# Kamino666/S2VT-video-caption

Hardware: AMD Instinct MI355X
Metric: training frames/sec (whole node) (higher is better)
Workload: dtype f32; 1 GPU; BASELINE configs[1]: S2VT train step, B=64 per GPU x 1 GPU, 80x4096 feats, hidden=embed=1000, vocab=12000, fp32, Adam; global_batch=64, frames=80, parallelism=dp1

## Files before the change

### s2vt-video-caption_amd/csrc/api_train.hip

```cpp
#include "api_internal.h"

namespace s2vt {

struct TrainWS : TrainBufs {
    float* colsum_c;
    float* ce_alpha;
    unsigned int *psync_a, *psync_b;
    unsigned short *xw1, *xw2, *xh1, *xh2;
    int64_t xkp;
    bool xfwd;
    unsigned short *xwt1, *xwt2;
    float *xpart1, *xpart2;
    int xnslots; int64_t xpslot, xhp;
    size_t bytes;
};

static TrainWS carve_train(const s2vt_dims& d, void* base) {
    const size_t B = d.B, L = d.L, H = d.H, E = d.E, V = d.V, T = 2 * L - 1;
    Carver c{reinterpret_cast<char*>(base), 0, 0};
    TrainWS w;
    w.bsum1 = c.take<float>(4 * H);
    w.bsum2 = c.take<float>(4 * H);
    w.x1 = c.take<float>(L * B * H);
    w.s1 = c.take<float>(T * B * 4 * H);
    w.h1 = c.take<float>(T * B * H);
    w.c1 = c.take<float>(T * B * H);
    w.s2 = c.take<float>(T * B * 4 * H);
    w.h2 = c.take<float>(T * B * H);
    w.c2 = c.take<float>(T * B * H);
    w.tok = c.take<int32_t>((L - 1) * B);
    w.embws = c.take<int>(embedding_grad_ws_ints((int64_t)(L - 1) * B, (int)d.V));
    w.err = c.take<int>(4);
    w.psync_a = c.take<unsigned int>(lstm_persist_sync_bytes() / sizeof(unsigned int));
    w.psync_b = c.take<unsigned int>(lstm_persist_sync_bytes() / sizeof(unsigned int));
    w.xkp = (H <= 1024) ? (int64_t)((H + 63) / 64 * 64) : 0;
    w.xfwd = w.xkp > 0 && gemm_mode() == 3 && B % 64 == 0 && pipe_block() > 0 && persist_x3_fwd_on();
    w.xw1 = c.take<unsigned short>(w.xfwd ? 3 * 4 * H * w.xkp : 0);
    w.xw2 = c.take<unsigned short>(w.xfwd ? 3 * 4 * H * w.xkp : 0);
    w.xh1 = c.take<unsigned short>(w.xfwd ? 3 * T * B * w.xkp : 0);
    w.xh2 = c.take<unsigned short>(w.xfwd ? 3 * T * B * w.xkp : 0);
    {
        const bool can = w.xkp > 0 && B % 32 == 0 && pipe_block() > 0 && option(O_PERSIST_X3_BWD) != 0 && persist_on() &&
                         (option(O_PERSIST_X3_BWD) == 1 || B * cdiv((int)H, 16) / 32 * 2 <= 256);
        const size_t maxblk = (size_t)pipe_block() < T ? (size_t)pipe_block() : T;
        w.xnslots = can ? (int)maxblk + 1 : 0;
        w.xhp = (int64_t)((H + 15) / 16 * 16);
        w.xpslot = can ? (int64_t)lstm_seq_bwd_x3_part_slot_floats((int)B, (int)H) : 0;
        w.xwt1 = c.take<unsigned short>(can ? 3 * (size_t)w.xkp * 4 * w.xhp : 0);
        w.xwt2 = c.take<unsigned short>(can ? 3 * (size_t)w.xkp * 4 * w.xhp : 0);
        w.xpart1 = c.take<float>((size_t)w.xnslots * w.xpslot);
        w.xpart2 = c.take<float>((size_t)w.xnslots * w.xpslot);
    }
    w.wt1 = c.take<float>(H * 4 * H);
    w.wt2 = c.take<float>(H * 4 * H);
    w.dh1 = c.take<float>(T * B * H);
    w.dh2dec = c.take<float>((L - 1) * B * H);
    w.dx1 = c.take<float>(L * B * H);
    w.de = c.take<float>((L - 1) * B * E);
    w.dc1 = c.take<float>(B * H);
    w.dc2 = c.take<float>(B * H);
    w.ce_alpha = c.take<float>(64);
    size_t cs = 2 * colsum_partial_floats((int64_t)T * B, (int)(4 * H));
    size_t cs2 = colsum_partial_floats((int64_t)(L - 1) * B, (int)V);
    size_t cs3 = colsum_partial_floats((int64_t)L * B, (int)H);
    const size_t csm = cs > cs2 ? (cs > cs3 ? cs : cs3) : (cs2 > cs3 ? cs2 : cs3);
    w.colsum_a = c.take<float>(csm);
    w.colsum_b = c.take<float>(csm);
    w.colsum_c = c.take<float>(csm);
    w.gws_floats = gemm_ws_floats(d);
    w.gws_a = c.take<float>(w.gws_floats);
    w.gws_b = c.take<float>(w.gws_floats);
    w.bytes = align_up(c.off, 256);
    return w;
}

static hipEvent_t g_grad_ev[2] = {nullptr, nullptr};
static bool g_grad_ev_set[2] = {false, false};
static int g_bwd_persist_launches = 0, g_bwd_group0_after = 0;
void backward_order_reset() { g_bwd_persist_launches = g_bwd_group0_after = 0; }
int grads_ready(int group, hipStream_t s) {
    if (group == 0) {
        g_bwd_group0_after = g_bwd_persist_launches;
        cu_reserve_window(true);
    }
    if (!g_grad_ev[group]) S2VT_HIP(hipEventCreateWithFlags(&g_grad_ev[group], hipEventDisableTiming));
    if (!graph_capturing()) S2VT_HIP(hipEventRecord(g_grad_ev[group], s));
    g_grad_ev_set[group] = true;
    return 0;
}

struct PlaneWS {
    PB feats, wf, x1, wih1, h1, we, wv, emb, h2r, wo, whh1, whh2;
    PB dlog, woT, wvT, weT, wih1T, dg2, dg1, whh1T, whh2T;
    PB h2decB;
    size_t bytes;
};

static PlaneWS carve_planes(const s2vt_dims& d, int planes, void* base) {
    const size_t B = d.B, L = d.L, F = d.F, H = d.H, E = d.E, V = d.V, T = 2 * L - 1, R = (L - 1) * B;
    Carver c{reinterpret_cast<char*>(base), 0, 0};
    auto mk = [&](size_t rows, size_t k) { return take_planes(c, rows, k, planes); };
    PlaneWS w;
    w.feats = mk(B * L, F);   w.wf = mk(H, F);       w.x1 = mk(L * B, H);    w.wih1 = mk(4 * H, H);
    w.h1 = mk(T * B, H);      w.we = mk(4 * H, E);   w.wv = mk(4 * H, H);    w.emb = mk(R, E);
    w.h2r = mk(T * B, H);     w.wo = mk(V, H);
    if (planes == 1) {
        w.whh1 = mk(4 * H, H); w.whh2 = mk(4 * H, H); w.whh1T = mk(H, 4 * H); w.whh2T = mk(H, 4 * H);
    }
    w.dlog = mk(R, V);        w.woT = mk(H, V);
    w.wvT = mk(H, 4 * H);     w.weT = mk(E, 4 * H);  w.wih1T = mk(H, 4 * H);
    w.dg2 = mk(T * B, 4 * H); w.dg1 = mk(T * B, 4 * H);
    w.h2decB = mk(R, H);
    w.bytes = align_up(c.off, 256);
    return w;
}

struct FwdRecord { s2vt_dims d; int gemm_mode, planes, persist, blk; bool dlog_ready; };
static RecordTable<FwdRecord> g_fwd_records;
static void record_forward(const void* ws, const s2vt_dims& d, bool planes) {
    g_fwd_records.put(ws, FwdRecord{d, gemm_mode(), planes ? train_planes() : 0, persist_bits(), pipe_block(), false});
}
static int check_forward_record(const void* ws, const s2vt_dims& d, bool planes, bool* dlog_ready = nullptr) {
    FwdRecord r;
    S2VT_REQUIRE(g_fwd_records.take(ws, &r), "s2vt_train_backward: no s2vt_train_forward has run on this workspace");
    if (dlog_ready) *dlog_ready = r.dlog_ready;
    S2VT_REQUIRE(memcmp(&r.d, &d, sizeof(d)) == 0, "s2vt_train_backward: dims differ from the forward that filled this workspace");
    S2VT_REQUIRE(r.gemm_mode == gemm_mode() && r.planes == (planes ? train_planes() : 0) && r.persist == persist_bits() && r.blk == pipe_block(),
                 "s2vt_train_backward: the forward ran with gemm mode %d / recurrence options %d / pipeline block %d, now %d / %d / %d: the "
                 "workspace layout differs (do not change gemm_mode / persist / persist_x3_fwd / persist_x3_bwd / pipe_block "
                 "between a forward and its backward)", r.gemm_mode, r.persist, r.blk, gemm_mode(), persist_bits(), pipe_block());
    return 0;
}

static void key_options(std::vector<uint64_t>& key) {
    for (int i = 0; i < O_COUNT; ++i) key.push_back((uint64_t)(uint32_t)option(i));
    key.push_back((uint64_t)(uint32_t)cu_plan_cap_current());
    key.push_back((uint64_t)g_lane_delay_lanes);
    key.push_back((uint64_t)g_lane_delay_us);
}

struct BpttDone {
    int bias_chunk = 64;
    int hh1_t0 = 0;
    long word_grads_ev = -1;
    long demb_ev = -1;
};

struct TrainDriver : Lanes {
    const s2vt_params* p; const s2vt_grads* g; const TrainWS& w; const PlaneWS& q;
    const float* out_mask; float* logits;
    const int B, L, F, H, E, V, T, R, blk;
    const int64_t BH, B4H;
    const bool bf;
    const bool emit;
    std::vector<int> bd;
    TrainDriver(const s2vt_dims* d, const s2vt_params* p_, const s2vt_grads* g_, const TrainWS& w_, const PlaneWS& q_,
                const float* out_mask_, float* logits_)
        : p(p_), g(g_), w(w_), q(q_), out_mask(out_mask_), logits(logits_), B(d->B), L(d->L), F(d->F), H(d->H), E(d->E), V(d->V),
          T(2 * d->L - 1), R((d->L - 1) * d->B), blk(pipe_block()), BH((int64_t)d->B * d->H), B4H(4 * (int64_t)d->B * d->H),
          bf(q_.h1.planes == 1), emit(d->H % 8 == 0) {}
    int open_lanes(hipStream_t caller) { return open(caller, w.gws_a, w.gws_b, w.gws_floats, w.colsum_a, w.colsum_b); }
    void set_bounds(bool persistent) { bd = pipe_bounds(T, L, persistent ? balanced_block(L, blk) : blk); }

    int zero_k16(const PB& img, size_t first, size_t elems) {
        S2VT_HIP(hipMemset2DAsync(img.p + first, (size_t)64 * img.ld * 2, 0, elems * 2, (size_t)(T * B / 64), st));
        return 0;
    }
    int vid_half_gemm(const Lane& ln, int t0, int t1) {
        const bool cap = t0 >= L;
        return pgemm(ln, (t1 - t0) * B, 4 * H, H, q.h1, t0 * B, 0, q.wv, 0, 0, w.s2 + t0 * B4H, 4 * H, ID, cap ? nullptr : w.bsum2, cap);
    }
    int logits_gemm(const Lane& ln, int first_step) {
        const PB* a = &q.h2r;
        int a0 = L * B, rc;
        if (out_mask) {
            if ((rc = mul_vectors(ln.s, w.h2 + (int64_t)L * B * H, out_mask, w.dh2dec, (int64_t)R * H))) return rc;
            a = &q.h2decB; a0 = 0;
            if ((rc = psplit(ln, *a, a0, w.dh2dec, H, ID, R, H))) return rc;
        }
        return pgemm(ln, R - first_step * B, V, H, *a, a0 + first_step * B, 0, q.wo, 0, 0, logits + (int64_t)first_step * V, V, perm(B, L - 1),
                     p->out_b, false);
    }
    int fwd_x3_persistent(int f_cus, int tenths, int gxe_c);
    int fwd_bf16_persistent();
    int fwd_two_lanes();

    int split_dg_block(const Lane& ln, int layer, int t0, int t1, bool want_planes) {
        const PB& dg = layer == 2 ? q.dg2 : q.dg1;
        const float* in = (layer == 2 ? w.s2 : w.s1) + t0 * B4H;
        float* colpart = (layer == 2 ? w.colsum_a : w.colsum_b) + (int64_t)(t0 * B / 64) * 4 * H;
        return want_planes ? pdual(ln, in, 4 * H, ID, (t1 - t0) * B, 4 * H, &dg, t0 * B, nullptr, t0 * B, colpart)
                           : pcolpart(ln, dg.planes, in, 4 * H, ID, (t1 - t0) * B, 4 * H, colpart);
    }
    int dh1_gemm(const Lane& ln, int t0, int t1) {
        return pgemm(ln, (t1 - t0) * B, H, 4 * H, q.dg2, t0 * B, 0, q.wvT, 0, 0, w.dh1 + t0 * BH, H, ID, nullptr, false);
    }
    int word_weight_grads(const Lane& ln) {
        int rc;
        if ((rc = pgemm_tt(ln, 4 * H, H, (T - 1) * B, q.dg2, B, q.h2r, 0, g->word_w_hh, H, ID, nullptr, false))) return rc;
        if ((rc = pgemm_tt(ln, 4 * H, H, T * B, q.dg2, 0, q.h1, 0, g->word_w_ih + E, E + H, ID, nullptr, false))) return rc;
        return pgemm_tt(ln, 4 * H, E, R, q.dg2, L * B, q.emb, 0, g->word_w_ih, E + H, ID, nullptr, false);
    }
    int demb_gemm(const Lane& ln) { return pgemm(ln, R, E, 4 * H, q.dg2, L * B, 0, q.weT, 0, 0, w.de, E, ID, nullptr, false); }
    SeqBwdX3Args bwd_x3_args(int layer, int t0, int t1) {
        const bool word = layer == 2;
        SeqBwdX3Args a = word ? persist_bwd_x3_args(T, t0, t1, B, H, w.xkp, w.xhp, w.xwt2, w.dh2dec, L, w.c2, w.s2, w.dc2, w.xpart2, w.xpslot,
                                                    w.xnslots, w.psync_a, w.err + 1)
                              : persist_bwd_x3_args(T, t0, t1, B, H, w.xkp, w.xhp, w.xwt1, w.dh1, 0, w.c1, w.s1, w.dc1, w.xpart1, w.xpslot,
                                                    w.xnslots, w.psync_b, w.err + 1);
        if (emit) {
            a.dgp = word ? q.dg2.p : q.dg1.p; a.lddgp = word ? q.dg2.ld : q.dg1.ld;
            a.colpart = word ? w.colsum_a : w.colsum_b; a.skip_dg = 1;
        }
        return a;
    }
    int x3_bptt_begin();
    int bptt_x3_one_layer(int corun_cus, int corun_k, BpttDone* done);
    int bptt_x3_two_layer(int corun_cus, int corun_k, BpttDone* done);
    int bptt_bf16_persistent();
    int bptt_two_lanes();
};

int TrainDriver::fwd_x3_persistent(int f_cus, int tenths, int gxe_c) {
    int rc;
    if ((rc = hand(sx, st))) return rc;
    const int nb = (int)bd.size() - 1;
    for (const PB* img : {&q.h1, &q.h2r})
        if ((rc = zero_k16_tail(st, *img, H, (size_t)T * B))) return rc;
    int lg_c = (nb >= 2 && !out_mask) ? (L - 1) * ((2 * tenths + 1) / 3) / 10 : 0;
    if (lg_c > bd[nb - 1] - L) lg_c = bd[nb - 1] - L > 0 ? bd[nb - 1] - L : 0;
    for (int k = 0; k <= nb; ++k) {
        const bool hv = k < nb, hw = k >= 1;
        const bool co_first = k == 0 && nb >= 2 && gxe_c > 0, co_last = k == nb && lg_c > 0;
        if ((co_first || co_last) && (rc = hand(st, sx))) return rc;
        {
        ProfScope ps(st, K_STEP_FWD, (hv ? bd[k + 1] - bd[k] : 0) + (hw ? bd[k] - bd[k - 1] : 0));
        SeqFwdX3Args av, aw;
        if (hv) av = persist_fwd_x3_args(bd[k], bd[k + 1], B, H, T, w.xkp, w.s1, L, w.bsum1, w.xw1, w.xh1, w.h1, w.c1, w.psync_a, w.err + 1);
        if (hw) aw = persist_fwd_x3_args(bd[k - 1], bd[k], B, H, T, w.xkp, w.s2, T, w.bsum2, w.xw2, w.xh2, w.h2, w.c2, w.psync_b, w.err + 1);
        av.hblk = q.h1.p; av.ldhblk = q.h1.ld;
        aw.hblk = q.h2r.p; aw.ldhblk = q.h2r.ld;
        if (hv && hw) rc = lstm_seq_fwd_x3_persist2(st, av, &aw);
        else rc = lstm_seq_fwd_x3_persist2(st, hv ? av : aw, nullptr);
        }
        if (rc) return rc;
        if (co_first || co_last) {
            {
                CuPlanCap cap(f_cus);
                if (co_first)
                    rc = pgemm(lb, gxe_c, 4 * H, E, q.emb, R - gxe_c, 0, q.we, 0, 0, w.s2 + (int64_t)L * B4H + (int64_t)(R - gxe_c) * 4 * H, 4 * H,
                               ID, w.bsum2, false);
                else
                    rc = pgemm(lb, lg_c * B, V, H, q.h2r, L * B, 0, q.wo, 0, 0, logits, V, perm(B, L - 1), p->out_b, false);
            }
            if (rc || (rc = hand(sx, st))) return rc;
        }
        if (hv && (rc = vid_half_gemm(la, bd[k], bd[k + 1]))) return rc;
    }
    return logits_gemm(la, lg_c);
}

int TrainDriver::fwd_bf16_persistent() {
    int rc;
    if ((rc = hand(sx, st))) return rc;
    const int nb = (int)bd.size() - 1;
    for (int k = 0; k <= nb; ++k) {
        const bool hv = k < nb, hw = k >= 1;
        SeqFwdBf16Args av, aw;
        if (hv) av = persist_fwd_args(bd[k], bd[k + 1], B, H, w.s1, L, w.bsum1, q.whh1, q.h1, w.h1, w.c1, w.psync_a, w.err + 1);
        if (hw) aw = persist_fwd_args(bd[k - 1], bd[k], B, H, w.s2, T, w.bsum2, q.whh2, q.h2r, w.h2, w.c2, w.psync_b, w.err + 1);
        {
            ProfScope ps(st, K_STEP_FWD, (hv ? bd[k + 1] - bd[k] : 0) + (hw ? bd[k] - bd[k - 1] : 0));
            if (hv && hw) rc = lstm_seq_fwd_bf16_persist2(st, av, &aw);
            else rc = lstm_seq_fwd_bf16_persist2(st, hv ? av : aw, nullptr);
            if (rc) return rc;
        }
        if (hv && (rc = vid_half_gemm(la, bd[k], bd[k + 1]))) return rc;
    }
    return logits_gemm(la, 0);
}

int TrainDriver::fwd_two_lanes() {
    int rc;
    for (size_t k = 0; k + 1 < bd.size(); ++k) {
        const int t0 = bd[k], t1 = bd[k + 1];
        rc = bf ? seq_fwd_bf16(st, t0, t1, B, H, w.s1, L, w.bsum1, q.whh1, q.h1, w.h1, w.c1)
                : seq_fwd(st, t0, t1, B, H, w.s1, L, w.bsum1, p->vid_w_hh, w.h1, w.c1, true);
        if (rc) return rc;
        if ((rc = hand(st, sx))) return rc;
        if ((rc = pdual(lb, w.h1 + t0 * BH, H, ID, (t1 - t0) * B, H, bf ? nullptr : &q.h1, t0 * B, nullptr, t0 * B, nullptr))) return rc;
        if ((rc = vid_half_gemm(lb, t0, t1))) return rc;
        rc = bf ? seq_fwd_bf16(sx, t0, t1, B, H, w.s2, T, w.bsum2, q.whh2, q.h2r, w.h2, w.c2)
// ... 8 lines not shown
static int train_forward_x3(const s2vt_dims* d, const s2vt_params* p, const float* feats, const int64_t* targets,
                            int64_t targets_ld, float* logits, const TrainWS& w, const PlaneWS& q, hipStream_t st,
                            const float* out_mask) {
    TrainDriver x(d, p, nullptr, w, q, out_mask, logits);
    const int B = x.B, L = x.L, F = x.F, H = x.H, E = x.E, V = x.V, T = x.T, R = x.R;
    const int64_t B4H = x.B4H;
    int rc;
    if ((rc = x.open_lanes(st))) return rc;
    const hipStream_t sx = x.sx;
    const Lane &la = x.la, &lb = x.lb;
    const bool bf = x.bf;
    if ((rc = bias_sums(st, p, H, w.bsum1, w.bsum2))) return rc;
    if ((rc = fill_zero(st, w.err, 4 * sizeof(int)))) return rc;
    if ((rc = targets_to_time_major(st, targets, B, L - 1, targets_ld, V, w.tok, w.err))) return rc;
    if (bf) {
        if ((rc = zero_pad_cols_u16(st, q.h1.p, (int64_t)T * B, q.h1.ld, H, q.h1.kpad))) return rc;
        if ((rc = zero_pad_cols_u16(st, q.h2r.p, (int64_t)T * B, q.h2r.ld, H, q.h2r.kpad))) return rc;
        if ((rc = pdual(la, p->vid_w_hh, H, ID, 4 * H, H, &q.whh1, 0, &q.whh1T, 0, nullptr))) return rc;
    }
    if ((rc = x.hand(st, sx))) return rc;
    if (bf && (rc = pdual(lb, p->word_w_hh, H, ID, 4 * H, H, &q.whh2, 0, &q.whh2T, 0, nullptr))) return rc;
    RecKind kind = train_recurrence_plan(B, H).fwd;
    if (kind == REC_X3_PERSIST && !w.xfwd) kind = REC_PER_STEP;
    if (kind == REC_BF16_PERSIST && !persist_fwd_ok(B, H, q.whh1, q.h1)) kind = REC_PER_STEP;
    const bool px3_fwd = kind == REC_X3_PERSIST;
    if (px3_fwd) {
        if ((rc = split3_rows(sx, p->vid_w_hh, H, 4 * H, H, (int)w.xkp, w.xw1, 4 * (int64_t)H * w.xkp))) return rc;
        if ((rc = split3_rows(sx, p->word_w_hh, H, 4 * H, H, (int)w.xkp, w.xw2, 4 * (int64_t)H * w.xkp))) return rc;
    }
    if ((rc = pdual(lb, p->word_w_ih, E + H, ID, 4 * H, E, &q.we, 0, &q.weT, 0, nullptr))) return rc;
    if ((rc = pdual(lb, p->word_w_ih + E, E + H, ID, 4 * H, H, &q.wv, 0, &q.wvT, 0, nullptr))) return rc;
    if ((rc = pdual(lb, p->out_w, H, ID, V, H, &q.wo, 0, &q.woT, 0, nullptr))) return rc;
    if ((rc = pdual(lb, p->emb_w, E, gather(w.tok), R, E, &q.emb, 0, nullptr, 0, nullptr))) return rc;
    const int f_wgs = px3_fwd ? lstm_seq_fwd_x3_persist_single_workgroups(B, H) : 0;
    const int f_cus = f_wgs > 0 ? (planned_compute_units() - f_wgs - 2) / 8 * 8 : 0;
    const bool stages3 = px3_fwd && pipe_bounds(T, L, balanced_block(L, x.blk)).size() >= 3;
    const int tenths = (stages3 && sx != st && f_cus >= 64 && R >= 2560 && B % 64 == 0) ? option(O_CORUN) : 0;
    const int gxe_c = (R / 64 * (2 * tenths < 8 ? 2 * tenths : 8) / 10) * 64;
    if ((rc = pgemm(lb, R - gxe_c, 4 * H, E, q.emb, 0, 0, q.we, 0, 0, w.s2 + (int64_t)L * B4H, 4 * H, ID, w.bsum2, false))) return rc;
    if ((rc = psplit(la, q.feats, 0, feats, F, ID, B * L, F))) return rc;
    if ((rc = psplit(la, q.wf, 0, p->feat_w, F, ID, H, F))) return rc;
    if ((rc = pdual(la, p->vid_w_ih, H, ID, 4 * H, H, &q.wih1, 0, &q.wih1T, 0, nullptr))) return rc;
    if ((rc = pgemm(la, B * L, H, F, q.feats, 0, 0, q.wf, 0, 0, w.x1, H, perm(L, B), p->feat_b, false))) return rc;
    if ((rc = pdual(la, w.x1, H, ID, L * B, H, &q.x1, 0, nullptr, 0, nullptr))) return rc;
    if ((rc = pgemm(la, L * B, 4 * H, H, q.x1, 0, 0, q.wih1, 0, 0, w.s1, 4 * H, ID, w.bsum1, false))) return rc;
    x.set_bounds(kind != REC_PER_STEP);
    switch (kind) {
    case REC_X3_PERSIST: return x.fwd_x3_persistent(f_cus, tenths, gxe_c);
    case REC_BF16_PERSIST: return x.fwd_bf16_persistent();
    default: return x.fwd_two_lanes();
    }
}

int TrainDriver::x3_bptt_begin() {
    int rc;
    if ((rc = split3_wt(st, w.wt2, H, (int)w.xkp, (int)w.xhp, w.xwt2, w.xkp * 4 * w.xhp))) return rc;
    if ((rc = split3_wt(sx, w.wt1, H, (int)w.xkp, (int)w.xhp, w.xwt1, w.xkp * 4 * w.xhp))) return rc;
    if ((rc = hand(sx, st))) return rc;
    if (emit && q.dg2.kpad > 4 * H) {
        const size_t kc0 = (size_t)(4 * H / 16);
        for (const PB* img : {&q.dg2, &q.dg1}) {
            if ((rc = zero_k16_tail(st, *img, 4 * H, (size_t)T * B))) return rc;
            if (4 * H % 16)
                for (int pl = 0; pl < 3; ++pl)
                    if ((rc = zero_k16(*img, kc0 * K16_REC_ELEMS + (pl * 2 + 1) * K16_HALF_ELEMS, K16_HALF_ELEMS))) return rc;
        }
    }
    return 0;
}

int TrainDriver::bptt_x3_one_layer(int corun_cus, int corun_k, BpttDone* done) {
    int rc;
    const int nb = (int)bd.size() - 1;
    if ((rc = hand(st, sx))) return rc;
    int wo_r = 0;
    auto wo_part = [&]() -> int {
        if (wo_r >= R) return 0;
        int kk = corun_k < R - wo_r ? corun_k : R - wo_r;
        if (R - wo_r - kk < 512) kk = R - wo_r;
        const int r = pgemm_tt(lb, V, H, kk, q.dlog, wo_r, q.h2decB, wo_r, g->out_w, H, ID, nullptr, wo_r > 0);
        wo_r += kk;
        return r;
    };
    std::vector<long> dh1_done((size_t)nb);
    long wo_done = 0;
    {
        CuPlanCap cap(corun_cus);
        for (int k = nb - 1; k >= 0; --k) {
            const int t0 = bd[k], t1 = bd[k + 1];
            {
                ProfScope ps(st, K_STEP_BWD, t1 - t0);
                if ((rc = lstm_seq_bwd_x3_persist2(st, bwd_x3_args(2, t0, t1), nullptr))) return rc;
                ++g_bwd_persist_launches;
            }
            if ((rc = wo_part())) return rc;
            if ((rc = hand(st, sx))) return rc;
            if (!emit && (rc = split_dg_block(lb, 2, t0, t1, true))) return rc;
            if ((rc = dh1_gemm(lb, t0, t1))) return rc;
            if ((rc = record(sx, &dh1_done[(size_t)k]))) return rc;
        }
        while (wo_r < R)
            if ((rc = wo_part())) return rc;
        if ((rc = record(sx, &wo_done))) return rc;
        if ((rc = word_weight_grads(lb))) return rc;
        if ((rc = record(sx, &done->word_grads_ev))) return rc;
        if ((rc = demb_gemm(lb))) return rc;
        if ((rc = record(sx, &done->demb_ev))) return rc;
    }
    const int kc = nb / 2;
    const int hh1_t0 = nb >= 4 ? bd[kc] : 0;
    for (int k = nb - 1; k >= 0; --k) {
        const int t0 = bd[k], t1 = bd[k + 1];
        if ((rc = wait(st, dh1_done[(size_t)k]))) return rc;
        ProfScope ps(st, K_STEP_BWD, t1 - t0);
        if ((rc = lstm_seq_bwd_x3_persist2(st, bwd_x3_args(1, t0, t1), nullptr))) return rc;
        ++g_bwd_persist_launches;
        if (!emit && (rc = split_dg_block(la, 1, t0, t1, true))) return rc;
        if (hh1_t0 > 0 && k == kc) {
            if ((rc = hand(st, sx))) return rc;
            CuPlanCap cap(corun_cus);
            if ((rc = pgemm_tt(lb, 4 * H, H, (T - hh1_t0) * B, q.dg1, hh1_t0 * B, q.h1, (hh1_t0 - 1) * B, g->vid_w_hh, H, ID, nullptr, false))) return rc;
        }
    }
    done->bias_chunk = emit ? 32 : 64;
    done->hh1_t0 = hh1_t0;
    if ((rc = wait(st, wo_done))) return rc;
    if ((rc = grads_ready(0, st))) return rc;
    return hand(st, sx);
}

int TrainDriver::bptt_x3_two_layer(int corun_cus, int corun_k, BpttDone* done) {
    int rc;
    const int nb = (int)bd.size() - 1;
    for (int k = nb - 1; k >= -1; --k) {
        const bool hw = k >= 0, hv = k + 1 <= nb - 1;
        const bool solo = corun_k && nb >= 2 && (k == nb - 1 || k == -1);
        if (solo && (rc = hand(st, sx))) return rc;
        {
            ProfScope ps(st, K_STEP_BWD, (hw ? bd[k + 1] - bd[k] : 0) + (hv ? bd[k + 2] - bd[k + 1] : 0));
            SeqBwdX3Args aw, av;
            if (hw) aw = bwd_x3_args(2, bd[k], bd[k + 1]);
            if (hv) av = bwd_x3_args(1, bd[k + 1], bd[k + 2]);
            if (hw && hv) rc = lstm_seq_bwd_x3_persist2(st, aw, &av);
            else rc = lstm_seq_bwd_x3_persist2(st, hw ? aw : av, nullptr);
            ++g_bwd_persist_launches;
            if (rc) return rc;
        }
        if (solo) {
            const int r0 = (k == nb - 1) ? 0 : corun_k;
            {
                CuPlanCap cap(corun_cus);
                if ((rc = pgemm_tt(lb, V, H, corun_k, q.dlog, r0, q.h2decB, r0, g->out_w, H, ID, nullptr, r0 > 0))) return rc;
            }
            if ((rc = hand(sx, st))) return rc;
        }
        if (hw) {
            if (!emit && (rc = split_dg_block(la, 2, bd[k], bd[k + 1], true))) return rc;
            if ((rc = dh1_gemm(la, bd[k], bd[k + 1]))) return rc;
        }
        if (hv && !emit && (rc = split_dg_block(la, 1, bd[k + 1], bd[k + 2], true))) return rc;
    }
    done->bias_chunk = emit ? 32 : 64;
    if (!corun_k && (rc = grads_ready(0, st))) return rc;
    if ((rc = hand(st, sx))) return rc;
    if (corun_k) {
        const bool two = nb >= 2;
        const int r0 = two ? 2 * corun_k : 0;
        if ((rc = pgemm_tt(lb, V, H, R - r0, q.dlog, r0, q.h2decB, r0, g->out_w, H, ID, nullptr, two))) return rc;
        if ((rc = grads_ready(0, sx))) return rc;
    }
    return 0;
}

int TrainDriver::bptt_bf16_persistent() {
    int rc;
    if ((rc = hand(sx, st))) return rc;
    const int nb = (int)bd.size() - 1;
    for (int k = nb - 1; k >= -1; --k) {
        const bool hw = k >= 0, hv = k + 1 <= nb - 1;
        SeqBwdBf16Args aw, av;
        if (hw) aw = seq_bwd_bf16_args(T, bd[k], bd[k + 1], B, H, q.whh2T, q.dg2, w.dh2dec, L, w.c2, w.s2, w.dc2, w.psync_a, w.err + 1);
        if (hv) av = seq_bwd_bf16_args(T, bd[k + 1], bd[k + 2], B, H, q.whh1T, q.dg1, w.dh1, 0, w.c1, w.s1, w.dc1, w.psync_b, w.err + 1);
        {
            ProfScope ps(st, K_STEP_BWD, (hw ? bd[k + 1] - bd[k] : 0) + (hv ? bd[k + 2] - bd[k + 1] : 0));
            if (hw && hv) rc = lstm_seq_bwd_bf16_persist2(st, aw, &av);
            else rc = lstm_seq_bwd_bf16_persist2(st, hw ? aw : av, nullptr);
            ++g_bwd_persist_launches;
            if (rc) return rc;
        }
        if (hw) {
            if ((rc = split_dg_block(la, 2, bd[k], bd[k + 1], false))) return rc;
            if ((rc = dh1_gemm(la, bd[k], bd[k + 1]))) return rc;
        }
        if (hv && (rc = split_dg_block(la, 1, bd[k + 1], bd[k + 2], false))) return rc;
    }
    if ((rc = grads_ready(0, st))) return rc;
    return hand(st, sx);
}

int TrainDriver::bptt_two_lanes() {
    int rc;
    for (size_t k = bd.size() - 1; k >= 1; --k) {
        const int t0 = bd[k - 1], t1 = bd[k];
        rc = bf ? seq_bwd_bf16(st, T, t0, t1, B, H, q.whh2T, w.dh2dec, L, w.c2, w.s2, q.dg2, w.dc2)
                : seq_bwd(st, T, t0, t1, B, H, w.wt2, w.dh2dec, L, w.c2, w.s2, w.dc2);
        if (rc) return rc;
        if ((rc = split_dg_block(la, 2, t0, t1, !bf))) return rc;
        if ((rc = dh1_gemm(la, t0, t1))) return rc;
        if ((rc = hand(st, sx))) return rc;
        rc = bf ? seq_bwd_bf16(sx, T, t0, t1, B, H, q.whh1T, w.dh1, 0, w.c1, w.s1, q.dg1, w.dc1)
                : seq_bwd(sx, T, t0, t1, B, H, w.wt1, w.dh1, 0, w.c1, w.s1, w.dc1);
        if (rc) return rc;
        if ((rc = split_dg_block(lb, 1, t0, t1, !bf))) return rc;
    }
    return 0;
}

static int train_backward_x3(const s2vt_dims* d, const s2vt_params* p, const float* feats, const float* dlogits,
                             const s2vt_grads* g, float* dfeats, const TrainWS& w, const PlaneWS& q, hipStream_t st,
                             const float* out_mask, bool dlog_ready) {
    TrainDriver x(d, p, g, w, q, out_mask, nullptr);
    const int B = x.B, L = x.L, F = x.F, H = x.H, E = x.E, V = x.V, T = x.T, R = x.R;
    const int64_t BH = x.BH;
    int rc;
    if ((rc = x.open_lanes(st))) return rc;
    const hipStream_t sx = x.sx;
    const Lane &la = x.la, &lb = x.lb;
    const bool bf = x.bf;
    if (bf) {
        if ((rc = zero_pad_cols_u16(st, q.dg2.p, (int64_t)T * B, q.dg2.ld, 4 * H, q.dg2.kpad))) return rc;
        if ((rc = zero_pad_cols_u16(st, q.dg1.p, (int64_t)T * B, q.dg1.ld, 4 * H, q.dg1.kpad))) return rc;
    }
    if ((rc = x.hand(st, sx))) return rc;
    if (!dlog_ready && (rc = pdual(la, dlogits, V, ID, R, V, &q.dlog, 0, nullptr, 0, w.colsum_c))) return rc;
    if ((rc = x.hand(st, sx))) return rc;
    if ((rc = pgemm(la, R, H, V, q.dlog, 0, 0, q.woT, 0, 0, w.dh2dec, H, perm(L - 1, B), nullptr, false))) return rc;
    const bool ce_pow2 = dlog_ready && bf;
    if (ce_pow2 && (rc = scale_by_device_scalar(st, w.dh2dec, (int64_t)R * H, w.ce_alpha))) return rc;
    if (out_mask && (rc = mul_vectors(st, w.dh2dec, out_mask, w.dh2dec, (int64_t)R * H))) return rc;
    if (!bf && (rc = transpose_f32(st, p->word_w_hh, 4 * H, H, w.wt2))) return rc;
    RecKind kind = train_recurrence_plan(B, H).bwd;
    if (kind == REC_BF16_PERSIST && q.dg2.kpad != q.whh2T.kpad) kind = REC_PER_STEP;
    if (kind == REC_X3_PERSIST && !(w.xnslots > (x.blk < T ? x.blk : T))) kind = REC_PER_STEP;
    const bool px3_bwd = kind == REC_X3_PERSIST;
    const int x3_ns = px3_bwd ? lstm_seq_bwd_x3_persist_supported(B, H) : 0;
    const int one_layer_wgs = x3_ns > 0 ? (B / (32 * x3_ns)) * cdiv(H, 16) : 1 << 20;
    const int corun_cus = (planned_compute_units() - one_layer_wgs - 2) / 8 * 8;
    const int corun_k = (px3_bwd && option(O_CORUN) && sx != st && corun_cus >= 64 && R >= 2560) ? (R / 64 * option(O_CORUN) / 10) * 64 : 0;
    {
        const float* h2dec = w.h2 + L * BH;
        if (out_mask) {
            if ((rc = mul_vectors(sx, w.h2 + L * BH, out_mask, w.dx1, (int64_t)R * H))) return rc;
            h2dec = w.dx1;
        }
        if ((rc = psplit(lb, q.h2decB, 0, h2dec, H, perm(L - 1, B), R, H))) return rc;
        if (!corun_k && (rc = pgemm_tt(lb, V, H, R, q.dlog, 0, q.h2decB, 0, g->out_w, H, ID, nullptr, false))) return rc;
        if (!corun_k && ce_pow2 && (rc = scale_by_device_scalar(sx, g->out_w, (int64_t)V * H, w.ce_alpha))) return rc;
    }
    if ((rc = lcolsum_finish(lb, w.colsum_c, cdiv(R, 64), V, g->out_b, false))) return rc;
    if (kind == REC_PER_STEP && (rc = grads_ready(0, sx))) return rc;
    if (!bf && (rc = transpose_f32(sx, p->vid_w_hh, 4 * H, H, w.wt1))) return rc;
    x.set_bounds(kind != REC_PER_STEP);
    BpttDone done;
    switch (kind) {
    case REC_X3_PERSIST:
        if ((rc = x.x3_bptt_begin())) return rc;
        if (corun_k > 0 && x.bd.size() >= 3 && option(O_BPTT_SOLO) != 0) rc = x.bptt_x3_one_layer(corun_cus, corun_k, &done);
        else rc = x.bptt_x3_two_layer(corun_cus, corun_k, &done);
        break;
    case REC_BF16_PERSIST: rc = x.bptt_bf16_persistent(); break;
    default: rc = x.bptt_two_lanes(); break;
    }
    if (rc) return rc;
    if (done.word_grads_ev < 0 && (rc = x.word_weight_grads(la))) return rc;
    if ((rc = lcolsum_finish(la, w.colsum_a, T * B / done.bias_chunk, 4 * H, g->word_b_ih, false))) return rc;
    S2VT_HIP(hipMemcpyAsync(g->word_b_hh, g->word_b_ih, sizeof(float) * 4 * H, hipMemcpyDeviceToDevice, st));
    if ((rc = done.demb_ev >= 0 ? x.wait(st, done.demb_ev) : x.demb_gemm(la))) return rc;
    if ((rc = embedding_grad(st, w.de, R, E, w.tok, V, g->emb_w, w.embws))) return rc;
    if (done.word_grads_ev >= 0 && (rc = x.wait(st, done.word_grads_ev))) return rc;
    if ((rc = grads_ready(1, st))) return rc;
    const int hh1_rows = ((done.hh1_t0 > 0 ? done.hh1_t0 : T) - 1) * B;
    if ((rc = pgemm_tt(lb, 4 * H, H, hh1_rows, q.dg1, B, q.h1, 0, g->vid_w_hh, H, ID, nullptr, done.hh1_t0 > 0))) return rc;
    if ((rc = pgemm_tt(lb, 4 * H, H, L * B, q.dg1, 0, q.x1, 0, g->vid_w_ih, H, ID, nullptr, false))) return rc;
    if ((rc = lcolsum_finish(lb, w.colsum_b, T * B / done.bias_chunk, 4 * H, g->vid_b_ih, false))) return rc;
    S2VT_HIP(hipMemcpyAsync(g->vid_b_hh, g->vid_b_ih, sizeof(float) * 4 * H, hipMemcpyDeviceToDevice, sx));
    if ((rc = pgemm(lb, L * B, H, 4 * H, q.dg1, 0, 0, q.wih1T, 0, 0, w.dx1, H, perm(B, L), nullptr, false))) return rc;
    if ((rc = pdual(lb, w.dx1, H, ID, L * B, H, &q.x1, 0, nullptr, 0, w.colsum_b))) return rc;
    if ((rc = pgemm_tt(lb, H, F, L * B, q.x1, 0, q.feats, 0, g->feat_w, F, ID, nullptr, false))) return rc;
    if ((rc = lcolsum_finish(lb, w.colsum_b, L * B / 64, H, g->feat_b, false))) return rc;
    if (dfeats && (rc = lgemm(lb, true, false, L * B, F, H, w.dx1, H, ID, p->feat_w, F, ID, dfeats, F, ID, nullptr, false))) return rc;
    return x.hand(sx, st);
}

}

using namespace s2vt;

extern "C" {

struct PadWS { float* feats; int64_t* targets; float* logits; float* mask; float* dfeats; size_t bytes; };
static PadWS carve_pad(const s2vt_dims& d, const s2vt_dims& dp, void* base) {
    const size_t Bp = dp.B, L = d.L, F = d.F, H = d.H, V = d.V;
    Carver c{reinterpret_cast<char*>(base), 0, 0};
    PadWS w;
    w.feats = c.take<float>(Bp * L * F);
    w.targets = c.take<int64_t>(Bp * (L - 1));
    w.logits = c.take<float>(Bp * (L - 1) * V);
    w.mask = c.take<float>((L - 1) * Bp * H);
    w.dfeats = c.take<float>(Bp * L * F);
    w.bytes = align_up(c.off, 256);
    return w;
}
static size_t train_core_bytes(const s2vt_dims& d) {
    size_t n = carve_train(d, nullptr).bytes;
    if (planes_ok(d)) n += carve_planes(d, train_planes(), nullptr).bytes;
    return n;
}

int32_t s2vt_padded_batch(int32_t B) {
    if (B <= 0) return 0;
    s2vt_dims d = {B, 2, 1, 1, 1, 1};
    return batch_padded(d) ? padded_dims(d).B : B;
}

size_t s2vt_train_workspace_bytes(const s2vt_dims* d) {
    if (!dims_ok(d)) return 0;
    if (batch_padded(*d)) {
        const s2vt_dims dp = padded_dims(*d);
        return align_up(train_core_bytes(dp), 256) + carve_pad(*d, dp, nullptr).bytes;
    }
    return train_core_bytes(*d);
}

static inline uint64_t kw(const void* p) { return (uint64_t)(uintptr_t)p; }
static std::vector<uint64_t> graph_key(uint64_t tag, const s2vt_dims* d, const s2vt_params* p, const s2vt_grads* g, std::initializer_list<uint64_t> words) {
    std::vector<uint64_t> key;
    if (!graph_on()) return key;
    key.reserve(80);
    key.push_back(tag);
    for (int v : {d->B, d->L, d->F, d->H, d->E, d->V}) key.push_back((uint64_t)v);
    key_options(key);
    const float* const* pp = reinterpret_cast<const float* const*>(p);
    for (size_t i = 0; i < sizeof(s2vt_params) / sizeof(void*); ++i) key_ptr(key, pp[i]);
    float* const* gp = reinterpret_cast<float* const*>(g);
    for (size_t i = 0; g && i < sizeof(s2vt_grads) / sizeof(void*); ++i) key_ptr(key, gp[i]);
    key.insert(key.end(), words);
    return key;
}

static int train_forward_core(const s2vt_dims* d, const s2vt_params* p, const float* feats, const int64_t* targets,
                              int64_t targets_ld, float* logits, void* workspace, size_t workspace_bytes, void* stream,
// ... 51 lines not shown
                               size_t workspace_bytes, void* stream) {
    return train_forward_impl(d, p, feats, targets, targets_ld, logits, workspace, workspace_bytes, stream, out_mask);
}

static int train_backward_core(const s2vt_dims* d, const s2vt_params* p, const float* feats, const float* dlogits,
                               const s2vt_grads* g, float* dfeats, void* workspace, size_t workspace_bytes, void* stream,
                               const float* out_mask) {
    BackwardScope scope;
    const TrainWS w = carve_train(*d, workspace);
    S2VT_REQUIRE(workspace_bytes >= w.bytes, "s2vt_train_backward: workspace %zu < %zu bytes", workspace_bytes, w.bytes);
    hipStream_t st = (hipStream_t)stream;
    bool dlog_ready = false;
    int rc0 = poll_async_error(false);
    if (rc0 || (rc0 = check_forward_record(workspace, *d, planes_ok(*d), &dlog_ready))) return rc0;
    S2VT_REQUIRE(dlogits || dlog_ready, "s2vt_train_backward: dlogits is null and s2vt_mean_ce_backward_fused has not run on this workspace");
    if (planes_ok(*d)) {
        const PlaneWS q = carve_planes(*d, train_planes(), reinterpret_cast<char*>(workspace) + w.bytes);
        S2VT_REQUIRE(workspace_bytes >= w.bytes + q.bytes, "s2vt_train_backward: workspace %zu < %zu bytes", workspace_bytes, w.bytes + q.bytes);
        const std::vector<uint64_t> key = graph_key(0xB0 + (dlog_ready ? 1 : 0), d, p, g, {kw(feats), kw(dlogits), kw(dfeats), kw(workspace),
                                                                                            kw(out_mask), kw(st)});
        bool graphed = false;
        rc0 = run_graphed(st, key, [&](hipStream_t s_) {
                LaneDelayScope delay(s_);
                return train_backward_x3(d, p, feats, dlogits, g, dfeats, w, q, s_, out_mask, dlog_ready);
            }, &graphed);
        if (!rc0 && graphed) {
            if ((rc0 = grads_ready(0, st))) return rc0;
            if ((rc0 = grads_ready(1, st))) return rc0;
        }
        return rc0 ? rc0 : post_async_error(st, w.err, 1);
    }
    return train_backward_f32(d, p, feats, dlogits, g, dfeats, w, st, out_mask);
}
static int train_backward_impl(const s2vt_dims* d, const s2vt_params* p, const float* feats, const float* dlogits,
                               const s2vt_grads* g, float* dfeats, void* workspace, size_t workspace_bytes, void* stream,
                               const float* out_mask) {
    S2VT_REQUIRE(dims_ok(d) && p && feats && g && workspace, "s2vt_train_backward: null/invalid argument");
    if (!batch_padded(*d)) return train_backward_core(d, p, feats, dlogits, g, dfeats, workspace, workspace_bytes, stream, out_mask);
    S2VT_REQUIRE(dlogits, "s2vt_train_backward: dlogits is null (the fused criterion backward needs a batch that is a multiple of 64)");
    const s2vt_dims dp = padded_dims(*d);
    const size_t core = align_up(train_core_bytes(dp), 256);
    const PadWS s = carve_pad(*d, dp, reinterpret_cast<char*>(workspace) + core);
    S2VT_REQUIRE(workspace_bytes >= core + s.bytes, "s2vt_train_backward: workspace %zu < %zu bytes", workspace_bytes, core + s.bytes);
    hipStream_t st = (hipStream_t)stream;
    const size_t B = d->B, Bp = dp.B, L = d->L, F = d->F, V = d->V;
    int rc;
    S2VT_HIP(hipMemcpyAsync(s.logits, dlogits, B * (L - 1) * V * sizeof(float), hipMemcpyDeviceToDevice, st));
    if ((rc = fill_zero(st, s.logits + B * (L - 1) * V, (Bp - B) * (L - 1) * V * sizeof(float)))) return rc;
    if ((rc = train_backward_core(&dp, p, s.feats, s.logits, g, dfeats ? s.dfeats : nullptr, workspace, core, stream, out_mask ? s.mask : nullptr))) return rc;
    if (dfeats) S2VT_HIP(hipMemcpyAsync(dfeats, s.dfeats, B * L * F * sizeof(float), hipMemcpyDeviceToDevice, st));
    return 0;
}

int s2vt_train_backward(const s2vt_dims* d, const s2vt_params* p, const float* feats, const float* dlogits,
                        const s2vt_grads* g, float* dfeats, void* workspace, size_t workspace_bytes, void* stream) {
    return train_backward_impl(d, p, feats, dlogits, g, dfeats, workspace, workspace_bytes, stream, nullptr);
}
int s2vt_train_backward_dropout(const s2vt_dims* d, const s2vt_params* p, const float* feats, const float* dlogits,
                                const float* out_mask, const s2vt_grads* g, float* dfeats, void* workspace,
                                size_t workspace_bytes, void* stream) {
    return train_backward_impl(d, p, feats, dlogits, g, dfeats, workspace, workspace_bytes, stream, out_mask);
}

int s2vt_backward_order(int32_t* persistent_bptt_launches, int32_t* group0_recorded_after) {
    if (persistent_bptt_launches) *persistent_bptt_launches = g_bwd_persist_launches;
    if (group0_recorded_after) *group0_recorded_after = g_bwd_group0_after;
    return 0;
}

int s2vt_backward_wait_grads(int32_t group, void* stream) {
    S2VT_REQUIRE(group == 0 || group == 1, "s2vt_backward_wait_grads: group must be 0 (out_linear) or 1 (word_rnn + embedding)");
    S2VT_REQUIRE(g_grad_ev_set[group], "s2vt_backward_wait_grads: no s2vt_train_backward has run yet");
    S2VT_HIP(hipStreamWaitEvent((hipStream_t)stream, g_grad_ev[group], 0));
    return 0;
}


int s2vt_mean_ce_backward_fused(const s2vt_dims* d, const float* logits, const int64_t* target, int64_t target_ld, const float* lse,
                                const float* gout, void* workspace, size_t workspace_bytes, void* stream) {
    S2VT_REQUIRE(dims_ok(d) && logits && target && lse && gout && workspace, "s2vt_mean_ce_backward_fused: null/invalid argument");
    S2VT_REQUIRE(planes_ok(*d), "s2vt_mean_ce_backward_fused: the workspace is not a plane-driver workspace (B %% 64, gemm mode 1 or 3)");
    const TrainWS w = carve_train(*d, workspace);
    S2VT_REQUIRE(g_fwd_records.with(workspace, [&](const FwdRecord& r) {
                     return memcmp(&r.d, d, sizeof(*d)) == 0 && r.gemm_mode == gemm_mode() && !r.dlog_ready;
                 }), "s2vt_mean_ce_backward_fused: no matching s2vt_train_forward has run on this workspace");
    const PlaneWS q = carve_planes(*d, train_planes(), reinterpret_cast<char*>(workspace) + w.bytes);
    S2VT_REQUIRE(workspace_bytes >= w.bytes + q.bytes, "s2vt_mean_ce_backward_fused: workspace %zu < %zu bytes", workspace_bytes, w.bytes + q.bytes);
    const int R = (d->L - 1) * d->B, V = d->V;
    CeGradArgs ce;
    ce.lse = lse; ce.target = target; ce.gout = gout; ce.Lm1 = d->L - 1; ce.ldt = target_ld;
    ce.alpha_out = (q.dlog.planes == 1) ? w.ce_alpha : nullptr;
    hipStream_t st = (hipStream_t)stream;
    int rc;
    {
        ProfScope ps(st, K_CE, 1);
        if ((rc = split_planes_dual(st, q.dlog.planes, logits, V, ID, R, V, q.dlog.p, q.dlog.ld, q.dlog.kpad, nullptr, 0, 0, w.colsum_c, &ce))) return rc;
    }
    g_fwd_records.with(workspace, [](FwdRecord& r) { return r.dlog_ready = true; });
    return 0;
}

}
```

### s2vt-video-caption_amd/csrc/common.h

```cpp
#pragma once
#include <hip/hip_runtime.h>
#include <stdint.h>
#include <stdio.h>

typedef float f32x4 __attribute__((ext_vector_type(4)));
typedef float f32x16 __attribute__((ext_vector_type(16)));

namespace s2vt {

void set_error(const char* fmt, ...);
int check_hip(hipError_t e, const char* what);

#define S2VT_HIP(call)                                        \
    do {                                                      \
        int _rc = ::s2vt::check_hip((call), #call);           \
        if (_rc) return _rc;                                  \
    } while (0)

#define S2VT_LAUNCH_CHECK(name)                               \
    do {                                                      \
        int _rc = ::s2vt::check_hip(hipGetLastError(), name); \
        if (_rc) return _rc;                                  \
    } while (0)

#define S2VT_REQUIRE(cond, ...)                               \
    do {                                                      \
        if (!(cond)) {                                        \
            ::s2vt::set_error(__VA_ARGS__);                   \
            return -1;                                        \
        }                                                     \
    } while (0)

static inline int cdiv(int a, int b) { return (a + b - 1) / b; }

enum Option { O_GEMM_MODE, O_PERSIST, O_PERSIST_X3_FWD, O_PERSIST_X3_BWD, O_PIPE_BLOCK, O_GRAPH, O_DECODE_FUSED, O_CU_RESERVE, O_BPTT_UNITS, O_GEMV, O_PAD_MIN_BATCH, O_CORUN, O_BPTT_SOLO, O_COUNT };
int option(int id);
int option_set(int id, int value);
int planned_compute_units();
int cu_plan_cap(int n);
int cu_plan_cap_current();
bool cu_reserve_window(bool on);
struct CuPlanCap {
    int prev;
    explicit CuPlanCap(int n) : prev(cu_plan_cap(n)) {}
    ~CuPlanCap() { cu_plan_cap(prev); }
};

int coresident_capacity(const void* kernel, int block);
static inline size_t align_up(size_t x, size_t a) { return (x + a - 1) / a * a; }

struct RowMap {
    const int32_t* idx;
    int inner, outer;
};

__device__ __forceinline__ int map_row(const RowMap& m, int r) {
    if (m.idx) return m.idx[r];
    if (m.inner) return (r % m.inner) * m.outer + r / m.inner;
    return r;
}

__device__ __forceinline__ int map_row_perm(const RowMap& m, int r) {
    const int inner = m.inner ? m.inner : 1;
    const int pr = (r % inner) * m.outer + r / inner;
    return m.inner ? pr : r;
}

static __device__ __attribute__((aligned(16))) float g_zero4[4] = {0.f, 0.f, 0.f, 0.f};

__device__ __forceinline__ float sigmoidf_(float x) { return 1.0f / (1.0f + __expf(-x)); }
__device__ __forceinline__ float tanhf_(float x) { return 1.0f - 2.0f / (1.0f + __expf(2.0f * x)); }

__device__ __forceinline__ unsigned short bf16_rn_bits(float x) {
    unsigned int u = __float_as_uint(x);
    if ((u & 0x7fffffffu) > 0x7f800000u) return (unsigned short)((u >> 16) | 0x40);
    u += 0x7fffu + ((u >> 16) & 1u);
    return (unsigned short)(u >> 16);
}
__device__ __forceinline__ void split3_bits(float x, unsigned short (&o)[3]) {
    o[0] = bf16_rn_bits(x);
    const float r1 = x - __uint_as_float((unsigned int)o[0] << 16);
    o[1] = bf16_rn_bits(r1);
    const float r2 = r1 - __uint_as_float((unsigned int)o[1] << 16);
    o[2] = bf16_rn_bits(r2);
}

}
```

### s2vt-video-caption_amd/csrc/options.hip

```cpp
#include <ctype.h>
#include <limits.h>
#include <stdlib.h>
#include <string.h>

#include "../../include/s2vt_hip.h"
#include "common.h"

namespace s2vt {

struct OptionDef { const char* name; int def, lo, hi; };
static const OptionDef kOptions[O_COUNT] = {
     {"gemm_mode", 3, 0, 3},
     {"persist", 1, 0, 1},
     {"persist_x3_fwd", 1, 0, 1},
     {"persist_x3_bwd", 2, 0, 2},
     {"pipe_block", 32, 0, 4096},
     {"graph", 0, 0, 1},
     {"decode_fused", 1, 0, 1},
     {"cu_reserve", 0, 0, 128},
     {"bptt_units", 0, 0, 32},
     {"gemv", 1, 0, 2},
     {"pad_min_batch", 33, 1, 64},
     {"corun", 3, 0, 5},
     {"bptt_solo", 1, 0, 1},
};
static int g_value[O_COUNT];
static bool g_read[O_COUNT];

static int clamp_to(const OptionDef& d, int v) { return v < d.lo ? d.lo : (v > d.hi ? d.hi : v); }

int option(int id) {
    if (id < 0 || id >= O_COUNT) return 0;
    if (!g_read[id]) {
        const OptionDef& d = kOptions[id];
        char env[64] = "S2VT_";
        size_t n = strlen(env);
        for (const char* c = d.name; *c && n + 1 < sizeof(env); ++c) env[n++] = (char)toupper((unsigned char)*c);
        env[n] = 0;
        const char* e = getenv(env);
        int v = d.def;
        if (e && *e) {
            v = atoi(e);
            if (id == O_GEMM_MODE && v != 1 && v != 3) v = 0;
            v = clamp_to(d, v);
        }
        g_value[id] = v;
        g_read[id] = true;
    }
    return g_value[id];
}

int option_set(int id, int value) {
    const int prev = option(id);
    if (id >= 0 && id < O_COUNT && value >= 0) {
        if (id == O_GEMM_MODE && value != 1 && value != 3) value = 0;
        g_value[id] = clamp_to(kOptions[id], value);
    }
    return prev;
}

static thread_local int t_cu_cap = 0;
static thread_local bool t_reserve_window = false;

bool cu_reserve_window(bool on) {
    const bool prev = t_reserve_window;
    t_reserve_window = on;
    return prev;
}

int planned_compute_units() {
    static int device_cus = 0;
    if (!device_cus) {
        int dev = 0, n = 0;
        if (hipGetDevice(&dev) != hipSuccess || hipDeviceGetAttribute(&n, hipDeviceAttributeMultiprocessorCount, dev) != hipSuccess || n < 8) n = 256;
        (void)hipGetLastError();
        device_cus = n;
    }
    int n = device_cus;
    const int reserve = t_reserve_window ? option(O_CU_RESERVE) : 0;
    if (reserve > 0 && reserve < n - 8) n -= reserve;
    if (t_cu_cap >= 8 && t_cu_cap < n) n = t_cu_cap;
    return n / 8 * 8;
}

int cu_plan_cap_current() { return t_cu_cap; }

int cu_plan_cap(int n) {
    const int prev = t_cu_cap;
    t_cu_cap = n > 0 ? n : 0;
    return prev;
}

int option_id(const char* name) {
    if (!name) return -1;
    for (int i = 0; i < O_COUNT; ++i)
        if (strcmp(name, kOptions[i].name) == 0) return i;
    return -1;
}

}

extern "C" {

int32_t s2vt_set_option(const char* name, int32_t value) {
    const int id = s2vt::option_id(name);
    if (id < 0) {
        s2vt::set_error("s2vt_set_option: unknown option '%s'", name ? name : "(null)");
// ... 10 lines not shown
```

Baseline: 504,300 frames/s.

## Use one joint partial-sum ring to enlarge one-layer BPTT blocks

Adds a bptt_block option and, in the solo one-layer BPTT path, treats the two layers' adjacent partial-sum rings as one joint ring. This allows larger time blocks (possibly the whole sequence), which means fewer persistent-kernel launches and handoffs. It also splits the output-projection weight-grad work into several parts for large blocks and moves the vid_w_hh co-run GEMM to start at the encoder/decoder boundary. The cost is less overlap granularity between the recurrence and the co-running GEMMs, and it relies on the two ring buffers being laid out contiguously in the workspace.

```diff
diff --git a/s2vt-video-caption_amd/csrc/api_train.hip b/s2vt-video-caption_amd/csrc/api_train.hip
--- a/s2vt-video-caption_amd/csrc/api_train.hip
+++ b/s2vt-video-caption_amd/csrc/api_train.hip
@@ -14,6 +14,26 @@
     int xnslots; int64_t xpslot, xhp;
     size_t bytes;
 };
+
+static int bptt_one_layer_block(int L, int ring_slots) {
+    const int n = option(O_BPTT_BLOCK);
+    if (n > 0) return n;
+    const int cap = ring_slots - 1;
+    if (cap >= L) return L;
+    if (cap < 1) return balanced_block(L, pipe_block());
+    const int nblk = (L + cap - 1) / cap;
+    return (L + nblk - 1) / nblk;
+}
+static int bptt_ring_slots(int B, int L) {
+    const int T = 2 * L - 1;
+    int slots = (pipe_block() < T ? pipe_block() : T) + 1;
+    const int n = option(O_BPTT_BLOCK);
+    if (n > 0 && gemm_mode() == 3 && option(O_CORUN) > 0 && option(O_BPTT_SOLO) != 0 && B % 64 == 0 && (int64_t)(L - 1) * B >= 2560) {
+        const int longest = n < L ? n : L;
+        if ((longest + 2) / 2 > slots) slots = (longest + 2) / 2;
+    }
+    return slots;
+}
 
 static TrainWS carve_train(const s2vt_dims& d, void* base) {
     const size_t B = d.B, L = d.L, H = d.H, E = d.E, V = d.V, T = 2 * L - 1;
@@ -42,8 +62,7 @@
     {
         const bool can = w.xkp > 0 && B % 32 == 0 && pipe_block() > 0 && option(O_PERSIST_X3_BWD) != 0 && persist_on() &&
                          (option(O_PERSIST_X3_BWD) == 1 || B * cdiv((int)H, 16) / 32 * 2 <= 256);
-        const size_t maxblk = (size_t)pipe_block() < T ? (size_t)pipe_block() : T;
-        w.xnslots = can ? (int)maxblk + 1 : 0;
+        w.xnslots = can ? bptt_ring_slots((int)B, (int)L) : 0;
         w.xhp = (int64_t)((H + 15) / 16 * 16);
         w.xpslot = can ? (int64_t)lstm_seq_bwd_x3_part_slot_floats((int)B, (int)H) : 0;
         w.xwt1 = c.take<unsigned short>(can ? 3 * (size_t)w.xkp * 4 * w.xhp : 0);
@@ -115,20 +134,22 @@
     return w;
 }
 
-struct FwdRecord { s2vt_dims d; int gemm_mode, planes, persist, blk; bool dlog_ready; };
+struct FwdRecord { s2vt_dims d; int gemm_mode, planes, persist, blk, bptt_blk; bool dlog_ready; };
 static RecordTable<FwdRecord> g_fwd_records;
 static void record_forward(const void* ws, const s2vt_dims& d, bool planes) {
-    g_fwd_records.put(ws, FwdRecord{d, gemm_mode(), planes ? train_planes() : 0, persist_bits(), pipe_block(), false});
+    g_fwd_records.put(ws, FwdRecord{d, gemm_mode(), planes ? train_planes() : 0, persist_bits(), pipe_block(), option(O_BPTT_BLOCK), false});
 }
 static int check_forward_record(const void* ws, const s2vt_dims& d, bool planes, bool* dlog_ready = nullptr) {
     FwdRecord r;
     S2VT_REQUIRE(g_fwd_records.take(ws, &r), "s2vt_train_backward: no s2vt_train_forward has run on this workspace");
     if (dlog_ready) *dlog_ready = r.dlog_ready;
     S2VT_REQUIRE(memcmp(&r.d, &d, sizeof(d)) == 0, "s2vt_train_backward: dims differ from the forward that filled this workspace");
-    S2VT_REQUIRE(r.gemm_mode == gemm_mode() && r.planes == (planes ? train_planes() : 0) && r.persist == persist_bits() && r.blk == pipe_block(),
-                 "s2vt_train_backward: the forward ran with gemm mode %d / recurrence options %d / pipeline block %d, now %d / %d / %d: the "
-                 "workspace layout differs (do not change gemm_mode / persist / persist_x3_fwd / persist_x3_bwd / pipe_block "
-                 "between a forward and its backward)", r.gemm_mode, r.persist, r.blk, gemm_mode(), persist_bits(), pipe_block());
+    S2VT_REQUIRE(r.gemm_mode == gemm_mode() && r.planes == (planes ? train_planes() : 0) && r.persist == persist_bits() && r.blk == pipe_block() &&
+                     r.bptt_blk == option(O_BPTT_BLOCK),
+                 "s2vt_train_backward: the forward ran with gemm mode %d / recurrence options %d / pipeline block %d / BPTT block %d, now "
+                 "%d / %d / %d / %d: the workspace layout differs (do not change gemm_mode / persist / persist_x3_fwd / persist_x3_bwd / "
+                 "pipe_block / bptt_block between a forward and its backward)", r.gemm_mode, r.persist, r.blk, r.bptt_blk, gemm_mode(),
+                 persist_bits(), pipe_block(), option(O_BPTT_BLOCK));
     return 0;
 }
 
@@ -153,6 +174,7 @@
     const int64_t BH, B4H;
     const bool bf;
     const bool emit;
+    bool one_ring = false;
     std::vector<int> bd;
     TrainDriver(const s2vt_dims* d, const s2vt_params* p_, const s2vt_grads* g_, const TrainWS& w_, const PlaneWS& q_,
                 const float* out_mask_, float* logits_)
@@ -202,12 +224,15 @@
         return pgemm_tt(ln, 4 * H, E, R, q.dg2, L * B, q.emb, 0, g->word_w_ih, E + H, ID, nullptr, false);
     }
     int demb_gemm(const Lane& ln) { return pgemm(ln, R, E, 4 * H, q.dg2, L * B, 0, q.weT, 0, 0, w.de, E, ID, nullptr, false); }
+    int joint_ring_slots() const { return w.xpslot > 0 ? (int)((w.xpart2 + (int64_t)w.xnslots * w.xpslot - w.xpart1) / w.xpslot) : 0; }
     SeqBwdX3Args bwd_x3_args(int layer, int t0, int t1) {
         const bool word = layer == 2;
-        SeqBwdX3Args a = word ? persist_bwd_x3_args(T, t0, t1, B, H, w.xkp, w.xhp, w.xwt2, w.dh2dec, L, w.c2, w.s2, w.dc2, w.xpart2, w.xpslot,
-                                                    w.xnslots, w.psync_a, w.err + 1)
-                              : persist_bwd_x3_args(T, t0, t1, B, H, w.xkp, w.xhp, w.xwt1, w.dh1, 0, w.c1, w.s1, w.dc1, w.xpart1, w.xpslot,
-                                                    w.xnslots, w.psync_b, w.err + 1);
+        float* part = one_ring ? w.xpart1 : (word ? w.xpart2 : w.xpart1);
+        const int nslots = one_ring ? joint_ring_slots() : w.xnslots;
+        SeqBwdX3Args a = word ? persist_bwd_x3_args(T, t0, t1, B, H, w.xkp, w.xhp, w.xwt2, w.dh2dec, L, w.c2, w.s2, w.dc2, part, w.xpslot,
+                                                    nslots, w.psync_a, w.err + 1)
+                              : persist_bwd_x3_args(T, t0, t1, B, H, w.xkp, w.xhp, w.xwt1, w.dh1, 0, w.c1, w.s1, w.dc1, part, w.xpslot,
+                                                    nslots, w.psync_b, w.err + 1);
         if (emit) {
             a.dgp = word ? q.dg2.p : q.dg1.p; a.lddgp = word ? q.dg2.ld : q.dg1.ld;
             a.colpart = word ? w.colsum_a : w.colsum_b; a.skip_dg = 1;
@@ -382,6 +407,8 @@
         wo_r += kk;
         return r;
     };
+    const int fb = balanced_block(L, blk);
+    auto wo_parts_of = [&](int steps) { return fb > 0 && steps > fb ? (steps + fb / 2) / fb : 1; };
     std::vector<long> dh1_done((size_t)nb);
     long wo_done = 0;
     {
@@ -393,7 +420,8 @@
                 if ((rc = lstm_seq_bwd_x3_persist2(st, bwd_x3_args(2, t0, t1), nullptr))) return rc;
                 ++g_bwd_persist_launches;
             }
-            if ((rc = wo_part())) return rc;
+            for (int i = wo_parts_of(t1 - t0); i > 0; --i)
+                if ((rc = wo_part())) return rc;
             if ((rc = hand(st, sx))) return rc;
             if (!emit && (rc = split_dg_block(lb, 2, t0, t1, true))) return rc;
             if ((rc = dh1_gemm(lb, t0, t1))) return rc;
@@ -407,8 +435,7 @@
         if ((rc = demb_gemm(lb))) return rc;
         if ((rc = record(sx, &done->demb_ev))) return rc;
     }
-    const int kc = nb / 2;
-    const int hh1_t0 = nb >= 4 ? bd[kc] : 0;
+    const int hh1_t0 = nb >= 2 ? L : 0;
     for (int k = nb - 1; k >= 0; --k) {
         const int t0 = bd[k], t1 = bd[k + 1];
         if ((rc = wait(st, dh1_done[(size_t)k]))) return rc;
@@ -416,7 +443,7 @@
         if ((rc = lstm_seq_bwd_x3_persist2(st, bwd_x3_args(1, t0, t1), nullptr))) return rc;
         ++g_bwd_persist_launches;
         if (!emit && (rc = split_dg_block(la, 1, t0, t1, true))) return rc;
-        if (hh1_t0 > 0 && k == kc) {
+        if (hh1_t0 > 0 && t0 == hh1_t0) {
             if ((rc = hand(st, sx))) return rc;
             CuPlanCap cap(corun_cus);
             if ((rc = pgemm_tt(lb, 4 * H, H, (T - hh1_t0) * B, q.dg1, hh1_t0 * B, q.h1, (hh1_t0 - 1) * B, g->vid_w_hh, H, ID, nullptr, false))) return rc;
@@ -565,8 +592,16 @@
     switch (kind) {
     case REC_X3_PERSIST:
         if ((rc = x.x3_bptt_begin())) return rc;
-        if (corun_k > 0 && x.bd.size() >= 3 && option(O_BPTT_SOLO) != 0) rc = x.bptt_x3_one_layer(corun_cus, corun_k, &done);
-        else rc = x.bptt_x3_two_layer(corun_cus, corun_k, &done);
+        if (corun_k > 0 && x.bd.size() >= 3 && option(O_BPTT_SOLO) != 0) {
+            const int joint = x.joint_ring_slots(), nblk = bptt_one_layer_block(L, joint);
+            if (joint > (nblk < L ? nblk : L)) {
+                x.bd = pipe_bounds(T, L, nblk);
+                x.one_ring = true;
+            }
+            rc = x.bptt_x3_one_layer(corun_cus, corun_k, &done);
+        } else {
+            rc = x.bptt_x3_two_layer(corun_cus, corun_k, &done);
+        }
         break;
     case REC_BF16_PERSIST: rc = x.bptt_bf16_persistent(); break;
     default: rc = x.bptt_two_lanes(); break;
@@ -784,7 +819,8 @@
     S2VT_REQUIRE(planes_ok(*d), "s2vt_mean_ce_backward_fused: the workspace is not a plane-driver workspace (B %% 64, gemm mode 1 or 3)");
     const TrainWS w = carve_train(*d, workspace);
     S2VT_REQUIRE(g_fwd_records.with(workspace, [&](const FwdRecord& r) {
-                     return memcmp(&r.d, d, sizeof(*d)) == 0 && r.gemm_mode == gemm_mode() && !r.dlog_ready;
+                     return memcmp(&r.d, d, sizeof(*d)) == 0 && r.gemm_mode == gemm_mode() && r.persist == persist_bits() &&
+                            r.blk == pipe_block() && r.bptt_blk == option(O_BPTT_BLOCK) && !r.dlog_ready;
                  }), "s2vt_mean_ce_backward_fused: no matching s2vt_train_forward has run on this workspace");
     const PlaneWS q = carve_planes(*d, train_planes(), reinterpret_cast<char*>(workspace) + w.bytes);
     S2VT_REQUIRE(workspace_bytes >= w.bytes + q.bytes, "s2vt_mean_ce_backward_fused: workspace %zu < %zu bytes", workspace_bytes, w.bytes + q.bytes);
diff --git a/s2vt-video-caption_amd/csrc/common.h b/s2vt-video-caption_amd/csrc/common.h
--- a/s2vt-video-caption_amd/csrc/common.h
+++ b/s2vt-video-caption_amd/csrc/common.h
@@ -33,7 +33,7 @@
 
 static inline int cdiv(int a, int b) { return (a + b - 1) / b; }
 
-enum Option { O_GEMM_MODE, O_PERSIST, O_PERSIST_X3_FWD, O_PERSIST_X3_BWD, O_PIPE_BLOCK, O_GRAPH, O_DECODE_FUSED, O_CU_RESERVE, O_BPTT_UNITS, O_GEMV, O_PAD_MIN_BATCH, O_CORUN, O_BPTT_SOLO, O_COUNT };
+enum Option { O_GEMM_MODE, O_PERSIST, O_PERSIST_X3_FWD, O_PERSIST_X3_BWD, O_PIPE_BLOCK, O_GRAPH, O_DECODE_FUSED, O_CU_RESERVE, O_BPTT_UNITS, O_GEMV, O_PAD_MIN_BATCH, O_CORUN, O_BPTT_SOLO, O_BPTT_BLOCK, O_COUNT };
 int option(int id);
 int option_set(int id, int value);
 int planned_compute_units();
diff --git a/s2vt-video-caption_amd/csrc/options.hip b/s2vt-video-caption_amd/csrc/options.hip
--- a/s2vt-video-caption_amd/csrc/options.hip
+++ b/s2vt-video-caption_amd/csrc/options.hip
@@ -23,6 +23,7 @@
      {"pad_min_batch", 33, 1, 64},
      {"corun", 3, 0, 5},
      {"bptt_solo", 1, 0, 1},
+     {"bptt_block", 0, 0, 4096},
 };
 static int g_value[O_COUNT];
 static bool g_read[O_COUNT];
```

Result: no change. 506,300 frames/s (median of 6 runs) (+0.4%).
